# laboshinl/loam_velodyne

Hardware: AMD Instinct MI355X
Metric: sweeps/sec (64-ring, 1M-pt map): feature extraction + odometry + scan-to-map registration (higher is better)
Workload: dtype f32

## Files before the change

### loam_velodyne_amd/csrc/features.hip

```cpp
#include "features.hpp"
#include "pinned_copy.hpp"
#include "scan.hpp"

namespace loamx {

__device__ inline float sqdiff3(const float4& a, const float4& b) {
  const float dx = a.x - b.x, dy = a.y - b.y, dz = a.z - b.z;
  return dx * dx + dy * dy + dz * dz;
}
__device__ inline float sqdiff3w(const float4& a, const float4& b, float wb) {
  const float dx = a.x - b.x * wb, dy = a.y - b.y * wb, dz = a.z - b.z * wb;
  return dx * dx + dy * dy + dz * dz;
}

struct RingLds {
  uint8_t* flags;
  float* c;
  uint32_t* sorted;
  int8_t* label;
};

__device__ inline void wave_lds_sync() { __builtin_amdgcn_fence(__ATOMIC_ACQ_REL, "workgroup"); }

__device__ inline void mark_as_picked(uint32_t scan_i, int cr, uint8_t* flags, const uint8_t* gaps, int lane) {
  bool brk = false;
  if (lane < cr) brk = gaps[scan_i + lane] != 0;
  else if (lane >= 32 && lane < 32 + cr) brk = gaps[scan_i - (lane - 32) - 1] != 0;
  const unsigned long long m = __ballot(brk);
  const uint32_t mf = (uint32_t)(m & 0xffffffffull), mb = (uint32_t)(m >> 32);
  const int nf = mf ? __builtin_ctz(mf) : cr;
  const int nb = mb ? __builtin_ctz(mb) : cr;
  if (lane == 0) flags[scan_i] = 1;
  if (lane < nf) flags[scan_i + lane + 1] = 1;
  if (lane >= 32 && lane - 32 < nb) flags[scan_i - (lane - 32) - 1] = 1;
  wave_lds_sync();
}

__device__ inline void mark_as_picked_split(uint32_t scan_i, int cr, uint8_t* flags, uint8_t* fwd, const uint8_t* gaps, int lane, uint32_t r_lo,
                                            uint32_t r_hi) {
  bool brk = false;
  if (lane < cr) brk = gaps[scan_i + lane] != 0;
  else if (lane >= 32 && lane < 32 + cr) brk = gaps[scan_i - (lane - 32) - 1] != 0;
  const unsigned long long m = __ballot(brk);
  const uint32_t mf = (uint32_t)(m & 0xffffffffull), mb = (uint32_t)(m >> 32);
  const int nf = mf ? __builtin_ctz(mf) : cr;
  const int nb = mb ? __builtin_ctz(mb) : cr;
  if (lane == 0) flags[scan_i] = 1;
  if (lane < nf) {
    const uint32_t t = scan_i + lane + 1;
    if (t < r_hi) flags[t] = 1;
    else fwd[t] = 1;
  }
  if (lane >= 32 && lane - 32 < nb) {
    const uint32_t t = scan_i - (lane - 32) - 1;
    if (t >= r_lo) flags[t] = 1;
  }
  wave_lds_sync();
}

__device__ inline void region_picks(const FeatParams& P, int cr, uint32_t rn, uint32_t rgsp, uint32_t rscan, const float* rc, const uint32_t* rsorted,
                                    int8_t* rlabel, uint8_t* flags, uint8_t* fwd, const uint8_t* gaps, uint32_t* outS, uint32_t* outLS, uint32_t* outF,
                                    uint32_t* cnt3, int lane) {
  const uint32_t r_lo = rscan, r_hi = rscan + rn;
  uint32_t nS = 0, nLS = 0, nF = 0;
  {
    int picked = 0;
    int pos = (int)rn;
    while (pos > 0 && picked < P.max_less_sharp) {
      const int kk = pos - 1 - lane;
      const bool in = kk >= 0;
      const uint32_t e = in ? rsorted[kk] : 0u;
      const float ce = in ? rc[e] : 0.f;
      const bool above = in && (ce > P.curv_thr);
      const bool ok = above && flags[rscan + e] == 0;
      const unsigned long long mok = __ballot(ok), mstop = __ballot(in && !above);
      const int fo = mok ? __builtin_ctzll(mok) : 64, fs = mstop ? __builtin_ctzll(mstop) : 64;
      if (fo < fs) {
        const uint32_t pe = __shfl(e, fo, 64);
        picked++;
        if (lane == 0) {
          if (picked <= P.max_sharp) {
            rlabel[pe] = 2;
            outS[nS] = rgsp + pe;
          } else {
            rlabel[pe] = 1;
          }
          outLS[nLS] = rgsp + pe;
        }
        if (picked <= P.max_sharp) nS++;
        nLS++;
        if (fwd) mark_as_picked_split(rscan + pe, cr, flags, fwd, gaps, lane, r_lo, r_hi);
        else mark_as_picked(rscan + pe, cr, flags, gaps, lane);
        pos = pos - 1 - fo;
      } else if (fs < 64) {
        break;
      } else {
        pos -= 64;
      }
    }
  }
  {
    int picked = 0;
    int pos = 0;
    while (pos < (int)rn && picked < P.max_flat) {
      const int kk = pos + lane;
      const bool in = kk < (int)rn;
      const uint32_t e = in ? rsorted[kk] : 0u;
      const float ce = in ? rc[e] : 0.f;
      const bool below = in && (ce < P.curv_thr);
      const bool ok = below && flags[rscan + e] == 0;
      const unsigned long long mok = __ballot(ok), mstop = __ballot(in && !below);
      const int fo = mok ? __builtin_ctzll(mok) : 64, fs = mstop ? __builtin_ctzll(mstop) : 64;
      if (fo < fs) {
        const uint32_t pe = __shfl(e, fo, 64);
        picked++;
        if (lane == 0) {
          rlabel[pe] = -1;
          outF[nF] = rgsp + pe;
        }
        nF++;
        if (fwd) mark_as_picked_split(rscan + pe, cr, flags, fwd, gaps, lane, r_lo, r_hi);
        else mark_as_picked(rscan + pe, cr, flags, gaps, lane);
        pos = pos + fo + 1;
      } else if (fs < 64) {
        break;
      } else {
        pos += 64;
      }
    }
  }
  if (lane == 0) { cnt3[0] = nS; cnt3[1] = nLS; cnt3[2] = nF; }
  wave_lds_sync();
}

template <int KPL>
__device__ inline void wave_sort_curvature(const float* __restrict__ c, uint32_t n, uint32_t* __restrict__ sorted, int lane) {
  unsigned long long a[KPL];
#pragma unroll
  for (int r = 0; r < KPL; r++) {
    const uint32_t e = (uint32_t)(r * 64 + lane);
    a[r] = e < n ? ((unsigned long long)__float_as_uint(c[e]) << 32) | e : ~0ull;
  }
  constexpr uint32_t N = 64u * KPL;
#pragma nounroll
  for (uint32_t k = 2; k <= N; k <<= 1) {
#pragma nounroll
    for (uint32_t j = k >> 1; j >= (uint32_t)KPL; j >>= 1) {
      const int pl = (int)(j / KPL);
      const bool lower = (lane & pl) == 0;
#pragma unroll
      for (int r = 0; r < KPL; r++) {
        const unsigned long long x = a[r];
        const unsigned long long y = __shfl_xor(x, pl, 64);
        const uint32_t i = (uint32_t)lane * KPL + (uint32_t)r;
// ... 141 lines not shown
        if (!(ep > sp) || ep - sp + 1 < (unsigned long long)cr) simple = 0;
      }
      s_simple = simple && !force_sequential;
    }
    float* c = (float*)(wave_base + wid * wave_bytes);
    uint32_t* sorted = (uint32_t*)(c + nmax);
    int8_t* label = (int8_t*)(sorted + nmax);
    for (int jb = 0; jb < nreg; jb += FEAT_WAVES) {
      const int j = jb + wid;
      uint32_t n = 0, gsp = 0, scan_sp = 0;
      if (j < nreg) {
        const unsigned long long sp = ((s0 + cr) * (unsigned long long)(nreg - j) + (e0 - cr) * (unsigned long long)j) / nreg;
        const unsigned long long ep = ((s0 + cr) * (unsigned long long)(nreg - 1 - j) + (e0 - cr) * (unsigned long long)(j + 1)) / nreg - 1;
        if (ep > sp) {
          n = (uint32_t)(ep - sp + 1);
          gsp = base + (uint32_t)sp;
          scan_sp = (uint32_t)(sp - s0);
        }
      }
      if (lane == 0) { reg_n[wid] = n; reg_gsp[wid] = gsp; reg_scan[wid] = scan_sp; }
      for (uint32_t e = lane; e < n; e += 64) {
        c[e] = curv_all[scan_sp + e];
        label[e] = 0;
      }
      if (lane < 4 && n) c[n + lane] = __builtin_inff();
      __syncthreads();
      FT_TS(1);
      if (sortP == 64) wave_sort_curvature<1>(c, n, sorted, lane);
      else if (sortP == 128) wave_sort_curvature<2>(c, n, sorted, lane);
      else if (sortP == 256) wave_sort_curvature<4>(c, n, sorted, lane);
      else if (sortP == 512) wave_sort_curvature<8>(c, n, sorted, lane);
      else if (wid < (int)nwaves) {
        unsigned long long* keys = (unsigned long long*)(wave_base + nwaves * wave_bytes + (size_t)wid * sortP * 8);
        for (uint32_t e = lane; e < sortP; e += 64)
          keys[e] = e < n ? ((unsigned long long)__float_as_uint(c[e]) << 32) | e : ~0ull;
        wave_lds_sync();
        for (uint32_t k = 2; k <= sortP; k <<= 1) {
          for (uint32_t j = k >> 1; j > 0; j >>= 1) {
            for (uint32_t t = lane; t < sortP / 2; t += 64) {
              const uint32_t i = ((t / j) * 2 * j) + (t % j), l = i + j;
              const unsigned long long a = keys[i], b = keys[l];
              const bool up = (i & k) == 0;
              if ((a > b) == up) { keys[i] = b; keys[l] = a; }
            }
            wave_lds_sync();
          }
        }
        for (uint32_t e = lane; e < n; e += 64) sorted[e] = (uint32_t)keys[e];
      }
      __syncthreads();
      FT_TS(2);
      if (s_simple) {
        const uint32_t rn = reg_n[wid];
        if (rn) {
          if (wid == 0 && jb > 0)
            for (uint32_t e = lane; e < (uint32_t)cr && e < rn; e += 64) flags[reg_scan[0] + e] |= fwd[reg_scan[0] + e];
          wave_lds_sync();
          region_picks(P, cr, rn, reg_gsp[wid], reg_scan[wid], c, sorted, label, flags, fwd, gaps, pickS + (size_t)j * P.max_sharp,
                       pickLS + (size_t)j * P.max_less_sharp, pickF + (size_t)j * P.max_flat, rcnt[j], lane);
        }
        __syncthreads();
        if (wid == 0) {
          for (int w = 1; w < FEAT_WAVES && jb + w < nreg; w++) {
            const uint32_t rn2 = reg_n[w], rscan2 = reg_scan[w], rgsp2 = reg_gsp[w];
            const float* rc = (const float*)(wave_base + w * wave_bytes);
            const uint32_t* rsorted = (const uint32_t*)(rc + nmax);
            int8_t* rlabel = (int8_t*)(rsorted + nmax);
            const bool hit = lane < cr && (uint32_t)lane < rn2 && fwd[rscan2 + lane] != 0 && rlabel[lane] != 0;
            if (__ballot(hit)) {
              for (uint32_t e = lane; e < rn2; e += 64) {
                flags[rscan2 + e] = flags0[rscan2 + e] | (e < (uint32_t)cr ? fwd[rscan2 + e] : (uint8_t)0);
                rlabel[e] = 0;
              }
              for (uint32_t e = lane; e < (uint32_t)cr; e += 64) fwd[rscan2 + rn2 + e] = 0;
              wave_lds_sync();
              region_picks(P, cr, rn2, rgsp2, rscan2, rc, rsorted, rlabel, flags, fwd, gaps, pickS + (size_t)(jb + w) * P.max_sharp,
                           pickLS + (size_t)(jb + w) * P.max_less_sharp, pickF + (size_t)(jb + w) * P.max_flat, rcnt[jb + w], lane);
            }
          }
        }
      } else if (wid == 0) {
        for (int w = 0; w < FEAT_WAVES && jb + w < nreg; w++) {
          const uint32_t rn2 = reg_n[w];
          if (rn2 == 0) continue;
          const float* rc = (const float*)(wave_base + w * wave_bytes);
          const uint32_t* rsorted = (const uint32_t*)(rc + nmax);
          int8_t* rlabel = (int8_t*)(rsorted + nmax);
          region_picks(P, cr, rn2, reg_gsp[w], reg_scan[w], rc, rsorted, rlabel, flags, nullptr, gaps, pickS + (size_t)(jb + w) * P.max_sharp,
                       pickLS + (size_t)(jb + w) * P.max_less_sharp, pickF + (size_t)(jb + w) * P.max_flat, rcnt[jb + w], lane);
        }
      }
      __syncthreads();
      FT_TS(3);
      for (uint32_t e = lane; e < n; e += 64) lf_valid[gsp + e] = label[e] <= 0 ? 1 : 0;
      __syncthreads();
    }
  }
  if (wid == 0 && len > 2u * cr + 1u) {
    uint32_t* lists[3] = {pickS, pickLS, pickF};
    const uint32_t per[3] = {(uint32_t)P.max_sharp, (uint32_t)P.max_less_sharp, (uint32_t)P.max_flat};
    uint32_t tot[3] = {0, 0, 0};
    for (int j = 0; j < nreg; j++) {
#pragma unroll
      for (int q = 0; q < 3; q++) {
        const uint32_t cnt = rcnt[j][q], src = (uint32_t)j * per[q];
        if (src != tot[q]) {
          for (uint32_t k0 = 0; k0 < cnt; k0 += 64) {
            const uint32_t k = k0 + lane;
            const uint32_t v = k < cnt ? lists[q][src + k] : 0u;
            wave_lds_sync();
            if (k < cnt) lists[q][tot[q] + k] = v;
            wave_lds_sync();
          }
        }
        tot[q] += cnt;
      }
    }
    nS = tot[0]; nLS = tot[1]; nF = tot[2];
  }
  if (tid == 0) {
    cntS[r] = nS;
    cntLS[r] = nLS;
    cntF[r] = nF;
    npick[0] = nS; npick[1] = nLS; npick[2] = nF;
  }
  __syncthreads();
  for (uint32_t k = tid; k < npick[0]; k += blockDim.x) slotS[(size_t)r * capS + k] = cloud[pickS[k]];
  for (uint32_t k = tid; k < npick[1]; k += blockDim.x) slotLS[(size_t)r * capLS + k] = cloud[pickLS[k]];
  for (uint32_t k = tid; k < npick[2]; k += blockDim.x) slotF[(size_t)r * capF + k] = cloud[pickF[k]];
  FT_TS(4);
}

struct FeatRingLds {
  uint32_t flag_bytes, nmax, sortP, nwaves;
  size_t bytes;
};
constexpr size_t FEAT_LDS_STATIC = 1024;
constexpr size_t FEAT_LDS_MAX = 160 * 1024 - FEAT_LDS_STATIC;
static_assert(sizeof(uint32_t) * (3 * FEAT_WAVES + 3 + 64 * 3) + sizeof(int) <= FEAT_LDS_STATIC, "k_feat_ring's static LDS");

static FeatRingLds feat_ring_lds(uint32_t max_len, const FeatParams& p) {
  FeatRingLds r;
  const size_t caps = (size_t)(p.max_sharp + p.max_less_sharp + p.max_flat) * p.n_regions;
  r.flag_bytes = (max_len + 15u) & ~15u;
  r.nmax = (max_len / (uint32_t)p.n_regions + 8u + 15u) & ~15u;
  r.sortP = 64;
  while (r.sortP < r.nmax) r.sortP <<= 1;
  r.nwaves = (uint32_t)std::min(p.n_regions, FEAT_WAVES);
  r.bytes = ((8 * (size_t)r.flag_bytes + 4 * caps + 15) & ~(size_t)15) + (size_t)r.nwaves * r.nmax * (4 + 4 + 1) +
            (r.sortP > 512 ? (size_t)r.nwaves * r.sortP * 8 : 0) + 16;
  return r;
}

constexpr int LFV_THREADS = 1024;
constexpr uint32_t LFV_MAX = 4096;

__global__ __launch_bounds__(LFV_THREADS) void k_feat_lf_voxel(const float4* __restrict__ cloud, const uint32_t* __restrict__ ring_off,
                                                               const uint8_t* __restrict__ lf_valid, float inv_leaf, uint32_t P,
                                                               float4* __restrict__ slots, uint32_t* __restrict__ cnt) {
  extern __shared__ __attribute__((aligned(16))) char smem[];
  unsigned long long* keys = (unsigned long long*)smem;
  __shared__ uint32_t sc[17];
  __shared__ int mm[6];
  __shared__ uint32_t s_wcnt[LFV_THREADS / 64][256];
  __shared__ uint32_t s_base[256];
  const uint32_t r = blockIdx.x, tid = threadIdx.x;
  const uint32_t s0 = ring_off[r], len = ring_off[r + 1] - s0;
  if (tid < 3) mm[tid] = 2147483647;
  else if (tid < 6) mm[tid] = -2147483647 - 1;
  for (uint32_t k = tid; k < P; k += LFV_THREADS) keys[k] = ~0ull;
  __syncthreads();
  uint32_t base = 0;
  for (uint32_t b = 0; b < len; b += LFV_THREADS) {
    const uint32_t i = b + tid;
    const uint32_t v = (i < len && lf_valid[s0 + i]) ? 1u : 0u;
    uint32_t total;
    const uint32_t ex = block_excl_scan(v, sc, total);
    if (v) keys[base + ex] = i;
    base += total;
  }
  const uint32_t m = base;
  __syncthreads();
  {
    int lo[3] = {2147483647, 2147483647, 2147483647}, hi[3] = {-2147483647 - 1, -2147483647 - 1, -2147483647 - 1};
    for (uint32_t j = tid; j < m; j += LFV_THREADS) {
      const float4 p = cloud[s0 + (uint32_t)keys[j]];
      const int c[3] = {(int)floorf(p.x * inv_leaf), (int)floorf(p.y * inv_leaf), (int)floorf(p.z * inv_leaf)};
#pragma unroll
      for (int a = 0; a < 3; a++) { lo[a] = min(lo[a], c[a]); hi[a] = max(hi[a], c[a]); }
    }
#pragma unroll
    for (int off = 32; off > 0; off >>= 1) {
#pragma unroll
      for (int a = 0; a < 3; a++) {
        lo[a] = min(lo[a], __shfl_xor(lo[a], off, 64));
        hi[a] = max(hi[a], __shfl_xor(hi[a], off, 64));
      }
    }
    if ((tid & 63u) == 0) {
#pragma unroll
      for (int a = 0; a < 3; a++) { atomicMin(&mm[a], lo[a]); atomicMax(&mm[3 + a], hi[a]); }
    }
  }
  __syncthreads();
  const long long dx = (long long)mm[3] - mm[0] + 1, dy = (long long)mm[4] - mm[1] + 1, dz = (long long)mm[5] - mm[2] + 1;
  const bool pass = m > 0 && (dx > 2147483647LL || dy > 2147483647LL || dx * dy > 2147483647LL || dz > 2147483647LL / (dx * dy) + 1 || dx * dy * dz > 2147483647LL);
  for (uint32_t j = tid; j < m; j += LFV_THREADS) {
    const uint32_t li = (uint32_t)keys[j];
    unsigned long long k;
    if (pass) {
      k = (unsigned long long)j;
    } else {
      const float4 p = cloud[s0 + li];
      const int jx = (int)floorf(p.x * inv_leaf), jy = (int)floorf(p.y * inv_leaf), jz = (int)floorf(p.z * inv_leaf);
      k = (unsigned long long)((long long)(jx - mm[0]) + (long long)(jy - mm[1]) * dx + (long long)(jz - mm[2]) * dx * dy);
    }
    keys[j] = (k << 12) | li;
  }
  __syncthreads();
  unsigned long long* kb[2] = {keys, (unsigned long long*)(smem + (size_t)P * 8)};
  uint32_t npass = 0;
  if (!pass && m > 1) {
    const unsigned long long top = (unsigned long long)(dx * dy * dz - 1);
    const uint32_t bits = top ? 64u - (uint32_t)__builtin_clzll(top) : 0u;
    npass = (bits + 7u) / 8u;
  }
  {
    const uint32_t lane = tid & 63u, wid = tid >> 6;
    const uint32_t per_wave = ((m + LFV_THREADS - 1) / LFV_THREADS) * 64u;
    for (uint32_t ps = 0; ps < npass; ps++) {
      const uint32_t shift = 12u + 8u * ps;
      const unsigned long long* src = kb[ps & 1];
      unsigned long long* dst = kb[(ps & 1) ^ 1];
      for (uint32_t e = tid; e < (LFV_THREADS / 64) * 256; e += LFV_THREADS) (&s_wcnt[0][0])[e] = 0u;
      __syncthreads();
      unsigned long long key[4];
      uint32_t rank[4];
#pragma unroll
      for (int j = 0; j < 4; j++) {
        const uint32_t i = wid * per_wave + (uint32_t)j * 64u + lane;
        const bool in = (uint32_t)j * 64u < per_wave && i < m;
        key[j] = in ? src[i] : ~0ull;
        const uint32_t d = (uint32_t)((key[j] >> shift) & 255ull);
        unsigned long long mt = __ballot(in);
#pragma unroll
        for (int b = 0; b < 8; b++) {
          const unsigned long long bal = __ballot((d >> b) & 1u);
          mt &= ((d >> b) & 1u) ? bal : ~bal;
        }
        const unsigned long long below = mt & ((1ull << lane) - 1ull);
        const int leader = __builtin_ctzll(mt | (1ull << 63));
        uint32_t old = 0u;
        if (in && (int)lane == leader) {
          old = s_wcnt[wid][d];
          s_wcnt[wid][d] = old + (uint32_t)__popcll(mt);
        }
        old = __shfl(old, leader, 64);
        rank[j] = old + (uint32_t)__popcll(below);
        __builtin_amdgcn_wave_barrier();
      }
      __syncthreads();
      uint32_t run = 0;
      if (tid < 256) {
#pragma unroll
        for (int w = 0; w < LFV_THREADS / 64; w++) { const uint32_t c = s_wcnt[w][tid]; s_wcnt[w][tid] = run; run += c; }
      }
      uint32_t tot;
      const uint32_t ex = block_excl_scan(run, sc, tot);
      if (tid < 256) s_base[tid] = ex;
      __syncthreads();
#pragma unroll
      for (int j = 0; j < 4; j++) {
        const uint32_t i = wid * per_wave + (uint32_t)j * 64u + lane;
        if ((uint32_t)j * 64u < per_wave && i < m) {
          const uint32_t d = (uint32_t)((key[j] >> shift) & 255ull);
          dst[s_base[d] + s_wcnt[wid][d] + rank[j]] = key[j];
        }
      }
      __syncthreads();
    }
    if (npass & 1u) {
      for (uint32_t j = tid; j < m; j += LFV_THREADS) keys[j] = kb[1][j];
      __syncthreads();
    }
  }
  float4* sp = (float4*)(smem + (size_t)P * 8);
  for (uint32_t j = tid; j < m; j += LFV_THREADS) sp[j] = cloud[s0 + (uint32_t)(keys[j] & 4095ull)];
  __syncthreads();
  uint32_t obase = 0;
  for (uint32_t b = 0; b < m; b += LFV_THREADS) {
    const uint32_t j = b + tid;
    const bool head = j < m && (j == 0 || (keys[j] >> 12) != (keys[j - 1] >> 12));
    uint32_t total;
    const uint32_t ex = block_excl_scan(head ? 1u : 0u, sc, total);
    if (head) {
      const unsigned long long vk = keys[j] >> 12;
      float sx = 0.f, sy = 0.f, sz = 0.f, si = 0.f;
      uint32_t e = j;
      do {
        const float4 p = sp[e];
        sx += p.x; sy += p.y; sz += p.z; si += p.w;
        e++;
      } while (e < m && (keys[e] >> 12) == vk);
      const float c = (float)(e - j);
      slots[s0 + obase + ex] = make_float4(sx / c, sy / c, sz / c, si / c);
    }
    obase += total;
  }
  if (tid == 0) cnt[r] = obase;
}

__device__ inline uint32_t rings_before(const uint32_t* __restrict__ c, uint32_t r, int lane) {
  uint32_t part = 0u;
  for (uint32_t i = (uint32_t)lane; i < r; i += 64u) part += c[i];
#pragma unroll
  for (int d = 32; d > 0; d >>= 1) part += (uint32_t)__shfl_xor((int)part, d, 64);
  return part;
}
__global__ __launch_bounds__(64) void k_feat_compact(const float4* __restrict__ s0, const float4* __restrict__ s1, const float4* __restrict__ s2,
                                                     const uint32_t* __restrict__ c0, const uint32_t* __restrict__ c1, const uint32_t* __restrict__ c2,
                                                     uint32_t cap0, uint32_t cap1, uint32_t cap2, float4* __restrict__ o0, float4* __restrict__ o1,
                                                     float4* __restrict__ o2, uint32_t* __restrict__ offs, const uint32_t* __restrict__ sweep_ring_base,
                                                     uint32_t nsw, uint32_t* __restrict__ host_offs) {
  const uint32_t r = blockIdx.x, kind = blockIdx.y, nring = gridDim.x;
  const int lane = (int)threadIdx.x;
  const float4* s = kind == 0 ? s0 : (kind == 1 ? s1 : s2);
  const uint32_t* c = kind == 0 ? c0 : (kind == 1 ? c1 : c2);
  const uint32_t cap = kind == 0 ? cap0 : (kind == 1 ? cap1 : cap2);
  float4* o = kind == 0 ? o0 : (kind == 1 ? o1 : o2);
  const uint32_t dst = rings_before(c, r, lane), n = c[r];
  for (uint32_t k = (uint32_t)lane; k < n; k += 64u) o[dst + k] = s[(size_t)r * cap + k];
  if (lane == 0) {
    uint32_t* off = offs + (size_t)kind * (nsw + 1);
    uint32_t* hoff = host_offs ? host_offs + (size_t)kind * (nsw + 1) : nullptr;
    uint32_t lo = 0, hi = nsw + 1;
    while (lo < hi) { const uint32_t mid = (lo + hi) >> 1; if (sweep_ring_base[mid] < r) lo = mid + 1; else hi = mid; }
    for (uint32_t sw = lo; sw <= nsw && sweep_ring_base[sw] == r; sw++) { off[sw] = dst; if (hoff) hoff[sw] = dst; }
    if (r + 1 == nring)
      for (uint32_t sw = nsw; sweep_ring_base[sw] >= nring; sw--) { off[sw] = dst + n; if (hoff) hoff[sw] = dst + n; if (sw == 0) break; }
  }
}
__global__ __launch_bounds__(256) void k_feat_lf_compact(const float4* __restrict__ slots, const uint32_t* __restrict__ ring_off,
                                                         const uint32_t* __restrict__ cnt, uint32_t* __restrict__ lf_off, float4* __restrict__ out,
                                                         uint32_t* __restrict__ host_lf_off) {
  __shared__ uint32_t s_dst;
  const uint32_t r = blockIdx.x;
  if (threadIdx.x < 64) {
    const uint32_t d = rings_before(cnt, r, (int)threadIdx.x);
    if (threadIdx.x == 0) {
      s_dst = d;
      lf_off[r] = d;
      if (r + 1 == gridDim.x) lf_off[gridDim.x] = d + cnt[r];
      if (host_lf_off) {
        host_lf_off[r] = d;
        if (r + 1 == gridDim.x) host_lf_off[gridDim.x] = d + cnt[r];
      }
    }
  }
  __syncthreads();
  const uint32_t n = cnt[r], src = ring_off[r], dst = s_dst;
  for (uint32_t k = threadIdx.x; k < n; k += blockDim.x) out[dst + k] = slots[src + k];
}

FeatureExtractor::FeatureExtractor(int device, hipStream_t shared_stream) : device_(device) {
  select_device(device);
  if (shared_stream) {
    st_ = shared_stream;
  } else {
    LX_HIP(hipStreamCreateWithFlags(&st_, hipStreamNonBlocking));
    own_stream_ = true;
  }
  vox_.init(st_);
  h_bad_.reserve(16);
  h_bad_.p[0] = 0u;
  h_bad_.p[1] = 0u;
}

void FeatureExtractor::check_finite_input() {
  if (*(volatile uint32_t*)h_bad_.p) {
    *h_bad_.p = 0u;
    throw Error(LOAMX_E_INVALID, "a sweep holds non-finite coordinates (binned rings must be finite: BasicLaserOdometry.cpp:230 / MultiScanRegistration.cpp:187-196 drop such points before this stage)");
  }
}

FeatureExtractor::~FeatureExtractor() {
  if (ev_front_) (void)hipEventDestroy(ev_front_);
  if (ev_lf_) (void)hipEventDestroy(ev_lf_);
  if (own_stream_ && st_) (void)hipStreamDestroy(st_);
}

void FeatureExtractor::check_params_() const {
  LX_REQUIRE(params.curv_region >= 1 && params.curv_region <= 16, "curvature_region must be in [1,16]");
  LX_REQUIRE(params.n_regions >= 1 && params.n_regions <= 64, "n_feature_regions must be in [1,64]");
  LX_REQUIRE(params.max_sharp >= 0 && params.max_flat >= 0 && params.max_less_sharp >= params.max_sharp, "invalid pick limits");
  LX_REQUIRE(params.less_flat_leaf > 0.f, "less_flat_filter_size must be positive");
}

void FeatureExtractor::upload_async(uint32_t nsw, const loamx_cloud* clouds, const uint32_t* const* ring_size, const uint32_t* n_rings,
                                    hipStream_t copy_stream, hipEvent_t done, const std::function<bool(void*, const void*, size_t)>& big_copy) {
  LX_REQUIRE(nsw >= 1 && clouds && ring_size && n_rings && copy_stream && done, "invalid sweep batch");
  check_params_();
  LX_HIP(hipSetDevice(device_));
  bool packed = true;
  for (uint32_t s = 0; s < nsw; s++) {
    check_cloud(&clouds[s], false);
    uint32_t sum = 0;
    for (uint32_t r = 0; r < n_rings[s]; r++) sum += ring_size[s][r];
    LX_REQUIRE(sum == clouds[s].count, "ring sizes do not add up to the cloud size");
    packed = packed && clouds[s].stride == 16 && clouds[s].intensity_offset == 12;
  }
  layout_(nsw, ring_size, n_rings);
  allocate_(copy_stream);
  if (packed) {
    for (uint32_t s = 0; s < nsw;) {
      uint32_t e = s + 1;
      size_t cnt = clouds[s].count;
      while (e < nsw && (const char*)clouds[e].data == (const char*)clouds[s].data + sizeof(float4) * cnt) cnt += clouds[e++].count;
      if (cnt && !(big_copy && big_copy(cloud_.p + h_pt_base_[s], clouds[s].data, sizeof(float4) * cnt)))
        LX_HIP(hipMemcpyAsync(cloud_.p + h_pt_base_[s], clouds[s].data, sizeof(float4) * cnt, hipMemcpyHostToDevice, copy_stream));
      s = e;
    }
  } else {
    h_cloud_.reserve(n_ + 1);
    for (uint32_t s = 0; s < nsw; s++) pack_cloud(&clouds[s], h_cloud_.p + h_pt_base_[s]);
    if (n_) LX_HIP(hipMemcpyAsync(cloud_.p, h_cloud_.p, sizeof(float4) * n_, hipMemcpyHostToDevice, copy_stream));
  }
  LX_HIP(hipEventRecord(done, copy_stream));
}
void FeatureExtractor::upload_device(uint32_t nsw, const float4* d_src, const uint32_t* src_off, const uint32_t* const* ring_size,
                                     const uint32_t* n_rings, hipStream_t copy_stream, hipEvent_t done) {
  LX_REQUIRE(nsw >= 1 && d_src && src_off && ring_size && n_rings && copy_stream && done, "invalid sweep batch");
  check_params_();
  LX_HIP(hipSetDevice(device_));
  layout_(nsw, ring_size, n_rings);
  allocate_(copy_stream);
  for (uint32_t s = 0; s < nsw; s++) {
    const uint32_t cnt = h_pt_base_[s + 1] - h_pt_base_[s];
    if (cnt) LX_HIP(hipMemcpyAsync(cloud_.p + h_pt_base_[s], d_src + src_off[s], sizeof(float4) * cnt, hipMemcpyDeviceToDevice, copy_stream));
  }
  LX_HIP(hipEventRecord(done, copy_stream));
}
void FeatureExtractor::layout_(uint32_t nsw, const uint32_t* const* ring_size, const uint32_t* n_rings) {
  uint32_t longest = 0;
  for (uint32_t s = 0; s < nsw; s++)
    for (uint32_t r = 0; r < n_rings[s]; r++) longest = std::max(longest, ring_size[s][r]);
  LX_REQUIRE(feat_ring_lds(longest, params).bytes <= FEAT_LDS_MAX, "scan ring too long for the LDS staging of k_feat_ring (include/loamx.h)");
  nsw_ = nsw;
  h_ring_off_.assign(1, 0);
  h_ring_base_.assign(nsw + 1, 0);
  h_pt_base_.assign(nsw + 1, 0);
  h_ring_sweep_base_.clear();
  max_ring_len_ = 0;
  uint32_t pt = 0;
  for (uint32_t s = 0; s < nsw; s++) {
    uint32_t sum = 0;
    for (uint32_t r = 0; r < n_rings[s]; r++) {
      sum += ring_size[s][r];
      h_ring_off_.push_back(pt + sum);
      h_ring_sweep_base_.push_back(pt);
      max_ring_len_ = std::max(max_ring_len_, ring_size[s][r]);
    }
    pt += sum;
// ... 123 lines not shown
    h_imu_d_.reserve(2 * (size_t)H);
    h_imu_f_.reserve(9 * (size_t)H);
    imu_.fill_table(h_imu_d_.p, h_imu_f_.p, I);
    imu_dt_.reserve(2 * (size_t)H);
    imu_state_.reserve(9 * (size_t)H);
    imu_last_.reserve(1);
    h_imu_last_.reserve(1);
    LX_HIP(hipMemcpyAsync(imu_dt_.p, h_imu_d_.p, sizeof(double) * 2 * H, hipMemcpyHostToDevice, st_));
    LX_HIP(hipMemcpyAsync(imu_state_.p, h_imu_f_.p, sizeof(float) * 9 * H, hipMemcpyHostToDevice, st_));
    LX_HIP(hipMemsetAsync(imu_last_.p, 0, sizeof(ImuLast), st_));
    I.dt = imu_dt_.p;
    I.dstamp = imu_dt_.p + H;
    I.state = imu_state_.p;
  }
  return H;
}

void FeatureExtractor::finish_raw_(uint32_t n_scan_rings, uint32_t H) {
  LX_HIP(hipMemcpyAsync(h_raw_ring_cnt_.p, raw_ring_cnt_.p, sizeof(uint32_t) * n_scan_rings, hipMemcpyDeviceToHost, st_));
  if (H) LX_HIP(hipMemcpyAsync(h_imu_last_.p, imu_last_.p, sizeof(ImuLast), hipMemcpyDeviceToHost, st_));
  LX_HIP(hipStreamSynchronize(st_));
  if (H && h_imu_last_.p->valid) imu_.apply_last(*h_imu_last_.p);
  begin_sweep();
  const uint32_t* rs[1] = {h_raw_ring_cnt_.p};
  layout_(1, rs, &n_scan_rings);
  allocate_();
  LX_HIP(hipStreamSynchronize(st_));
}

void ImuTracker::update(double stamp, float roll, float pitch, float yaw, const float acc_in[3]) {
  State st;
  st.stamp = stamp; st.roll = HAngle(roll); st.pitch = HAngle(pitch); st.yaw = HAngle(yaw);
  st.acceleration = {acc_in[0], acc_in[1], acc_in[2]};
  if (!hist_.empty()) {
    HVec3 acc = st.acceleration;
    h_rot_zxy(acc, st.roll, st.pitch, st.yaw);
    const State& prev = hist_.back();
    const float dt = (float)(stamp - prev.stamp);
    st.position = {prev.position.x + prev.velocity.x * dt + 0.5f * acc.x * dt * dt, prev.position.y + prev.velocity.y * dt + 0.5f * acc.y * dt * dt,
                   prev.position.z + prev.velocity.z * dt + 0.5f * acc.z * dt * dt};
    st.velocity = {prev.velocity.x + acc.x * dt, prev.velocity.y + acc.y * dt, prev.velocity.z + acc.z * dt};
  }
  if (hist_.size() >= (size_t)std::max(history_size, 1)) hist_.pop_front();
  hist_.push_back(st);
}

void ImuTracker::interpolate_for_(float rel, State& out) {
  double td = (scan_time_ - hist_[idx_].stamp) + rel;
  while (idx_ < hist_.size() - 1 && td > 0) {
    idx_++;
    td = (scan_time_ - hist_[idx_].stamp) + rel;
  }
  if (idx_ == 0 || td > 0) {
    out = hist_[idx_];
  } else {
    const State &a = hist_[idx_], &b = hist_[idx_ - 1];
    const float ratio = (float)(-td / (a.stamp - b.stamp)), inv = 1 - ratio;
    out.roll = HAngle(a.roll.r * inv + b.roll.r * ratio);
    out.pitch = HAngle(a.pitch.r * inv + b.pitch.r * ratio);
    if (a.yaw.r - b.yaw.r > M_PI) out.yaw = HAngle((float)(a.yaw.r * inv + (b.yaw.r + 2 * M_PI) * ratio));
    else if (a.yaw.r - b.yaw.r < -M_PI) out.yaw = HAngle((float)(a.yaw.r * inv + (b.yaw.r - 2 * M_PI) * ratio));
    else out.yaw = HAngle(a.yaw.r * inv + b.yaw.r * ratio);
    out.velocity = {a.velocity.x * inv + b.velocity.x * ratio, a.velocity.y * inv + b.velocity.y * ratio, a.velocity.z * inv + b.velocity.z * ratio};
    out.position = {a.position.x * inv + b.position.x * ratio, a.position.y * inv + b.position.y * ratio, a.position.z * inv + b.position.z * ratio};
  }
}

void ImuTracker::begin_sweep() {
  scan_time_ = next_scan_time_;
  idx_ = 0;
  if (!hist_.empty()) interpolate_for_(0.f, start_);
  sweep_start_ = scan_time_;
  imu_trans_[0] = start_.pitch.r; imu_trans_[1] = start_.yaw.r; imu_trans_[2] = start_.roll.r;
  imu_trans_[3] = cur_.pitch.r; imu_trans_[4] = cur_.yaw.r; imu_trans_[5] = cur_.roll.r;
  HVec3 sh = shift_;
  h_rot_yxz(sh, -start_.yaw, -start_.pitch, -start_.roll);
  imu_trans_[6] = sh.x; imu_trans_[7] = sh.y; imu_trans_[8] = sh.z;
  HVec3 v{cur_.velocity.x - start_.velocity.x, cur_.velocity.y - start_.velocity.y, cur_.velocity.z - start_.velocity.z};
  h_rot_yxz(v, -start_.yaw, -start_.pitch, -start_.roll);
  imu_trans_[9] = v.x; imu_trans_[10] = v.y; imu_trans_[11] = v.z;
}

void ImuTracker::fill_table(double* h_d, float* h_f, ImuTable& I) const {
  const uint32_t H = (uint32_t)hist_.size();
  for (uint32_t j = 0; j < H; j++) {
    const State& s = hist_[j];
    h_d[j] = scan_time_ - s.stamp;
    h_d[H + j] = j ? s.stamp - hist_[j - 1].stamp : 1.0;
    float* o = h_f + 9 * (size_t)j;
    o[0] = s.roll.r; o[1] = s.pitch.r; o[2] = s.yaw.r;
    o[3] = s.position.x; o[4] = s.position.y; o[5] = s.position.z;
    o[6] = s.velocity.x; o[7] = s.velocity.y; o[8] = s.velocity.z;
  }
  I.H = H;
  I.idx0 = H ? (uint32_t)std::min(idx_, (size_t)H - 1) : 0u;
  const HAngle* sa[3] = {&start_.roll, &start_.pitch, &start_.yaw};
  for (int k = 0; k < 3; k++) { I.start_c[k] = sa[k]->c; I.start_s[k] = sa[k]->s; }
  I.start_pos[0] = start_.position.x; I.start_pos[1] = start_.position.y; I.start_pos[2] = start_.position.z;
  I.start_vel[0] = start_.velocity.x; I.start_vel[1] = start_.velocity.y; I.start_vel[2] = start_.velocity.z;
  I.rel_sweep_base = scan_time_ - sweep_start_;
}

void ImuTracker::apply_last(const ImuLast& L) {
  cur_.roll = HAngle(L.roll); cur_.pitch = HAngle(L.pitch); cur_.yaw = HAngle(L.yaw);
  cur_.position = {L.pos[0], L.pos[1], L.pos[2]};
  cur_.velocity = {L.vel[0], L.vel[1], L.vel[2]};
  shift_ = {L.shift[0], L.shift[1], L.shift[2]};
  idx_ = L.idx;
}

int FeatureExtractor::download_cloud(uint32_t sweep, loamx_cloud* full, uint32_t* ring_size_out) {
  LX_REQUIRE(sweep < nsw_, "sweep index out of range");
  const uint32_t r0 = h_ring_base_[sweep], r1 = h_ring_base_[sweep + 1];
  if (ring_size_out)
    for (uint32_t r = r0; r < r1; r++) ring_size_out[r - r0] = h_ring_off_[r + 1] - h_ring_off_[r];
  if (!full) return LOAMX_OK;
  check_cloud(full, false);
  const uint32_t a = h_pt_base_[sweep], b = h_pt_base_[sweep + 1];
  h_pack_.reserve((size_t)(b - a) + 2);
  if (b > a) LX_HIP(hipMemcpyAsync(h_pack_.p, cloud_.p + a, sizeof(float4) * (b - a), hipMemcpyDeviceToHost, st_));
  LX_HIP(hipStreamSynchronize(st_));
  return unpack_cloud(h_pack_.p, b - a, full);
}

void FeatureExtractor::run_async(bool mirror_offsets) {
  TraceRange trace_range("loamx:features:extract");
  LX_REQUIRE(nsw_ > 0, "run() before upload()");
  LX_HIP(hipSetDevice(device_));
  split_ = mirror_offsets && max_ring_len_ <= LFV_MAX;
  uint32_t* hmir = nullptr;
  if (split_) {
    h_mirror_off_.reserve(n_offsets());
    hmir = h_mirror_off_.p;
    if (!ev_front_) { LX_HIP(hipEventCreateWithFlags(&ev_front_, hipEventDisableTiming)); LX_HIP(hipEventCreateWithFlags(&ev_lf_, hipEventDisableTiming)); }
  }
  const int cr = params.curv_region;
  (void)cr;
  const uint32_t caps[3] = {(uint32_t)(params.max_sharp * params.n_regions), (uint32_t)(params.max_less_sharp * params.n_regions),
                            (uint32_t)(params.max_flat * params.n_regions)};
  const FeatRingLds L = feat_ring_lds(max_ring_len_, params);
  const size_t lds = L.bytes;
  LX_REQUIRE(lds <= FEAT_LDS_MAX, "internal: scan ring too long for the LDS staging of k_feat_ring");
  static const bool force_seq = diag_env("LOAMX_FEAT_SEQUENTIAL") && atoi(diag_env("LOAMX_FEAT_SEQUENTIAL")) != 0;
  if (lds > 64 * 1024)
    LX_HIP(hipFuncSetAttribute((const void*)k_feat_ring, hipFuncAttributeMaxDynamicSharedMemorySize, (int)lds));
  hipLaunchKernelGGL(k_feat_ring, dim3(nring_), dim3(64 * FEAT_WAVES), lds, st_, cloud_.p, ring_off_.p, ring_sweep_base_.p, params, L.flag_bytes, L.nmax,
                     L.sortP, L.nwaves, slots_[0].p, slots_[1].p, slots_[2].p, slot_cnt_[0].p, slot_cnt_[1].p, slot_cnt_[2].p, lf_valid_.p, force_seq ? 1 : 0,
                     h_bad_.p);
  hipLaunchKernelGGL(k_feat_compact, dim3(nring_, 3), dim3(64), 0, st_, slots_[0].p, slots_[1].p, slots_[2].p, slot_cnt_[0].p, slot_cnt_[1].p,
                     slot_cnt_[2].p, caps[0], caps[1], caps[2], out_[0].p, out_[1].p, out_[2].p, offs_.p, sweep_ring_base_.p, nsw_, hmir);
  if (split_) LX_HIP(hipEventRecord(ev_front_, st_));
  const float inv = 1.0f / params.less_flat_leaf;
  if (max_ring_len_ <= LFV_MAX) {
    uint32_t P = 2;
    while (P < max_ring_len_) P <<= 1;
    if ((size_t)P * 24 > 64 * 1024)
      LX_HIP(hipFuncSetAttribute((const void*)k_feat_lf_voxel, hipFuncAttributeMaxDynamicSharedMemorySize, (int)((size_t)P * 24)));
    hipLaunchKernelGGL(k_feat_lf_voxel, dim3(nring_), dim3(LFV_THREADS), (size_t)P * 24, st_, cloud_.p, ring_off_.p, lf_valid_.p, inv, P,
                       lf_slots_.p, lf_cnt_.p);
    hipLaunchKernelGGL(k_feat_lf_compact, dim3(nring_), dim3(256), 0, st_, lf_slots_.p, ring_off_.p, lf_cnt_.p, lf_off_(), lf_out_.p,
                       hmir ? hmir + (size_t)3 * off_stride_ : nullptr);
    if (split_) LX_HIP(hipEventRecord(ev_lf_, st_));
  } else {
    vox_.compute_ijk(cloud_.p, lf_valid_.p, n_, ring_off_.p, nring_, inv, inv);
    vox_.sort_reduce(cloud_.p, lf_valid_.p, n_, ring_off_.p, nring_, lf_out_.p, lf_off_());
  }
#ifdef LOAMX_PROF_FEAT
  {
    unsigned long long ts[8];
    LX_HIP(hipStreamSynchronize(st_));
    LX_HIP(hipMemcpyFromSymbol(ts, HIP_SYMBOL(g_feat_ts), sizeof(ts)));
    fprintf(stderr, "[feat_ring ts, 10ns ticks] load %lld  rank-sort %lld  picks %lld  tail %lld\n", (long long)(ts[1] - ts[0]), (long long)(ts[2] - ts[1]),
            (long long)(ts[3] - ts[2]), (long long)(ts[4] - ts[3]));
  }
#endif
  LX_HIP(hipGetLastError());
}

void FeatureExtractor::sync() {
  LX_HIP(hipStreamSynchronize(st_));
  vox_.check();
  check_finite_input();
}

__global__ __launch_bounds__(256) void k_feat_pack_host(const float4* __restrict__ o0, const float4* __restrict__ o1, const float4* __restrict__ o2,
                                                        const float4* __restrict__ lf, const uint32_t* __restrict__ off0,
                                                        const uint32_t* __restrict__ off1, const uint32_t* __restrict__ off2,
                                                        const uint32_t* __restrict__ lf_off, uint32_t sweep, uint32_t ring_a, uint32_t ring_b,
                                                        uint32_t capacity, float4* __restrict__ dst) {
  const uint32_t a0 = off0[sweep], n0 = off0[sweep + 1] - a0, a1 = off1[sweep], n1 = off1[sweep + 1] - a1;
  const uint32_t a2 = off2[sweep], n2 = off2[sweep + 1] - a2, a3 = lf_off[ring_a], n3 = lf_off[ring_b] - a3;
  const uint32_t total = n0 + n1 + n2 + n3;
  if (blockIdx.x == 0 && threadIdx.x == 0) {
    uint4 h = make_uint4(n0, n1, n2, n3);
    if (total > capacity) h = make_uint4(0xffffffffu, 0xffffffffu, 0xffffffffu, 0xffffffffu);
    *reinterpret_cast<uint4*>(dst) = h;
  }
  if (total > capacity) return;
  for (uint32_t i = blockIdx.x * blockDim.x + threadIdx.x; i < total; i += gridDim.x * blockDim.x) {
    float4 v;
    if (i < n0) v = o0[a0 + i];
    else if (i < n0 + n1) v = o1[a1 + (i - n0)];
    else if (i < n0 + n1 + n2) v = o2[a2 + (i - n0 - n1)];
    else v = lf[a3 + (i - n0 - n1 - n2)];
    dst[1 + i] = v;
  }
}

void FeatureExtractor::device_results(uint32_t sweep, const float4* ptr[4], uint32_t count[4]) {
  LX_REQUIRE(sweep < nsw_, "sweep index out of range");
  h_link_off_.reserve(n_offsets());
  LX_HIP(hipMemcpyAsync(h_link_off_.p, offs_.p, sizeof(uint32_t) * n_offsets(), hipMemcpyDeviceToHost, st_));
  LX_HIP(hipStreamSynchronize(st_));
  vox_.check();
  check_finite_input();
  const uint32_t* o = h_link_off_.p;
  for (int k = 0; k < 3; k++) {
    const uint32_t a = o[(size_t)k * off_stride_ + sweep], b = o[(size_t)k * off_stride_ + sweep + 1];
    ptr[k] = out_[k].p + a;
    count[k] = b - a;
  }
  const uint32_t* lf = o + (size_t)3 * off_stride_;
  const uint32_t a = lf[h_ring_base_[sweep]], b = lf[h_ring_base_[sweep + 1]];
  ptr[3] = lf_out_.p + a;
  count[3] = b - a;
}

void FeatureExtractor::device_results_front(uint32_t sweep, const float4* ptr[3], uint32_t count[3]) {
  LX_REQUIRE(sweep < nsw_, "sweep index out of range");
  LX_REQUIRE(split_, "internal: device_results_front() without run_async(true)");
  spin_event(ev_front_);
  check_finite_input();
  const uint32_t* o = h_mirror_off_.p;
  for (int k = 0; k < 3; k++) {
    const uint32_t a = o[(size_t)k * off_stride_ + sweep], b = o[(size_t)k * off_stride_ + sweep + 1];
    ptr[k] = out_[k].p + a;
    count[k] = b - a;
  }
}
void FeatureExtractor::device_results_lf(uint32_t sweep, const float4*& ptr, uint32_t& count) {
  LX_REQUIRE(sweep < nsw_, "sweep index out of range");
  LX_REQUIRE(split_, "internal: device_results_lf() without run_async(true)");
  spin_event(ev_lf_);
  const uint32_t* lf = h_mirror_off_.p + (size_t)3 * off_stride_;
  const uint32_t a = lf[h_ring_base_[sweep]], b = lf[h_ring_base_[sweep + 1]];
  ptr = lf_out_.p + a;
  count = b - a;
}

int FeatureExtractor::download(uint32_t sweep, loamx_cloud* sharp, loamx_cloud* less_sharp, loamx_cloud* flat, loamx_cloud* less_flat) {
  LX_REQUIRE(sweep < nsw_, "sweep index out of range");
  loamx_cloud* outs[4] = {sharp, less_sharp, flat, less_flat};
  for (auto* o : outs) if (o) check_cloud(o, false);
  const uint32_t n_pts = h_pt_base_[sweep + 1] - h_pt_base_[sweep];
  const uint32_t capacity = 4 * n_pts;
  h_pack_.reserve((size_t)capacity + 2);
  hipLaunchKernelGGL(k_feat_pack_host, dim3(std::min<uint32_t>((capacity + 1023) / 1024 + 1, 128u)), dim3(256), 0, st_, out_[0].p, out_[1].p, out_[2].p,
                     lf_out_.p, d_feat_off(0), d_feat_off(1), d_feat_off(2), lf_off_(), sweep, h_ring_base_[sweep], h_ring_base_[sweep + 1], capacity,
                     h_pack_.p);
  LX_HIP(hipStreamSynchronize(st_));
  vox_.check();
  check_finite_input();
  const uint32_t* hdr = reinterpret_cast<const uint32_t*>(h_pack_.p);
  LX_REQUIRE(hdr[0] != 0xffffffffu, "internal: the feature clouds of a sweep exceed four times its points");
  int rc = LOAMX_OK;
  const float4* src = h_pack_.p + 1;
  for (int k = 0; k < 4; k++) {
    if (outs[k]) {
      const int r = unpack_cloud(src, hdr[k], outs[k]);
      if (r != LOAMX_OK) rc = r;
    }
    src += hdr[k];
  }
  return rc;
}

}
```

Measured before the change: 16240.

## Rework less-flat voxel kernel around register-resident keys and shared ring radix pass

Rewrites k_feat_lf_voxel so each thread holds eight points in registers. Points are loaded once into LDS staging, voxel coordinates are computed once, and keys stay in registers through each radix pass. A reusable ring_radix_pass uses 16-bit per-wave counters and a single-wave scan, and the block size is sized to the ring length (P/8, at most 512) rather than fixed at 1024. Voxel means are computed per thread over contiguous runs, with a tail walk for runs that cross thread boundaries. This cuts redundant global reloads, the compaction scan and barriers, at the cost of more complex boundary logic and an extra sort pass when all keys fit in one.

Measured after the change: 16610, median of 3. +2.3%, better.

```diff
diff --git a/loam_velodyne_amd/csrc/features.hip b/loam_velodyne_amd/csrc/features.hip
--- a/loam_velodyne_amd/csrc/features.hip
+++ b/loam_velodyne_amd/csrc/features.hip
@@ -1,5 +1,6 @@
 #include "features.hpp"
 #include "pinned_copy.hpp"
+#include "ring_radix.hpp"
 #include "scan.hpp"
 
 namespace loamx {
@@ -447,42 +448,60 @@
   return r;
 }
 
-constexpr int LFV_THREADS = 1024;
-constexpr uint32_t LFV_MAX = 4096;
-
-__global__ __launch_bounds__(LFV_THREADS) void k_feat_lf_voxel(const float4* __restrict__ cloud, const uint32_t* __restrict__ ring_off,
-                                                               const uint8_t* __restrict__ lf_valid, float inv_leaf, uint32_t P,
-                                                               float4* __restrict__ slots, uint32_t* __restrict__ cnt) {
+constexpr int LFV_MAX_THREADS = 512;
+constexpr uint32_t LFV_MAX = 4096, LFV_MIN_P = 512;
+static_assert(LFV_MAX / 8 == LFV_MAX_THREADS && LFV_MAX_THREADS / 64 <= RR_MAX_WAVES, "k_feat_lf_voxel: eight elements per thread");
+
+#ifdef LOAMX_PROF_LFV
+__device__ unsigned long long g_lfv_ts[8];
+#define LFV_TS(k) do { if (blockIdx.x == gridDim.x / 2 && threadIdx.x == 0) g_lfv_ts[k] = wall_clock64(); } while (0)
+#else
+#define LFV_TS(k) do { } while (0)
+#endif
+
+__global__ __launch_bounds__(LFV_MAX_THREADS) void k_feat_lf_voxel(const float4* __restrict__ cloud, const uint32_t* __restrict__ ring_off,
+                                                                   const uint8_t* __restrict__ lf_valid, float inv_leaf, uint32_t P,
+                                                                   float4* __restrict__ slots, uint32_t* __restrict__ cnt) {
   extern __shared__ __attribute__((aligned(16))) char smem[];
-  unsigned long long* keys = (unsigned long long*)smem;
+  float4* stage = (float4*)smem;
+  unsigned long long* s_w = (unsigned long long*)(smem + (size_t)P * 16);
+  __shared__ RingRadixLds s_rx;
   __shared__ uint32_t sc[17];
   __shared__ int mm[6];
-  __shared__ uint32_t s_wcnt[LFV_THREADS / 64][256];
-  __shared__ uint32_t s_base[256];
-  const uint32_t r = blockIdx.x, tid = threadIdx.x;
+  const uint32_t r = blockIdx.x, tid = threadIdx.x, lane = tid & 63u, wid = tid >> 6;
   const uint32_t s0 = ring_off[r], len = ring_off[r + 1] - s0;
   if (tid < 3) mm[tid] = 2147483647;
   else if (tid < 6) mm[tid] = -2147483647 - 1;
-  for (uint32_t k = tid; k < P; k += LFV_THREADS) keys[k] = ~0ull;
-  __syncthreads();
-  uint32_t base = 0;
-  for (uint32_t b = 0; b < len; b += LFV_THREADS) {
-    const uint32_t i = b + tid;
-    const uint32_t v = (i < len && lf_valid[s0 + i]) ? 1u : 0u;
-    uint32_t total;
-    const uint32_t ex = block_excl_scan(v, sc, total);
-    if (v) keys[base + ex] = i;
-    base += total;
-  }
-  const uint32_t m = base;
-  __syncthreads();
+  LFV_TS(0);
+  int vx[8], vy[8], vz[8];
+  uint32_t cand = 0u;
+  {
+    float4 pt[8];
+    uint8_t ok[8];
+#pragma unroll
+    for (int j = 0; j < 8; j++) {
+      const uint32_t i = wid * 512u + (uint32_t)j * 64u + lane;
+      pt[j] = i < len ? cloud[s0 + i] : make_float4(0.f, 0.f, 0.f, 0.f);
+      ok[j] = i < len ? lf_valid[s0 + i] : (uint8_t)0;
+    }
+#pragma unroll
+    for (int j = 0; j < 8; j++) {
+      const uint32_t i = wid * 512u + (uint32_t)j * 64u + lane;
+      if (i < len) stage[i] = pt[j];
+      cand |= ok[j] ? (1u << j) : 0u;
+      vx[j] = (int)floorf(pt[j].x * inv_leaf); vy[j] = (int)floorf(pt[j].y * inv_leaf); vz[j] = (int)floorf(pt[j].z * inv_leaf);
+    }
+  }
+  LFV_TS(1);
   {
     int lo[3] = {2147483647, 2147483647, 2147483647}, hi[3] = {-2147483647 - 1, -2147483647 - 1, -2147483647 - 1};
-    for (uint32_t j = tid; j < m; j += LFV_THREADS) {
-      const float4 p = cloud[s0 + (uint32_t)keys[j]];
-      const int c[3] = {(int)floorf(p.x * inv_leaf), (int)floorf(p.y * inv_leaf), (int)floorf(p.z * inv_leaf)};
-#pragma unroll
-      for (int a = 0; a < 3; a++) { lo[a] = min(lo[a], c[a]); hi[a] = max(hi[a], c[a]); }
+#pragma unroll
+    for (int j = 0; j < 8; j++) {
+      if ((cand >> j) & 1u) {
+        lo[0] = min(lo[0], vx[j]); hi[0] = max(hi[0], vx[j]);
+        lo[1] = min(lo[1], vy[j]); hi[1] = max(hi[1], vy[j]);
+        lo[2] = min(lo[2], vz[j]); hi[2] = max(hi[2], vz[j]);
+      }
     }
 #pragma unroll
     for (int off = 32; off > 0; off >>= 1) {
@@ -492,117 +511,112 @@
         hi[a] = max(hi[a], __shfl_xor(hi[a], off, 64));
       }
     }
-    if ((tid & 63u) == 0) {
+    __syncthreads();
+    if (lane == 0 && lo[0] <= hi[0]) {
 #pragma unroll
       for (int a = 0; a < 3; a++) { atomicMin(&mm[a], lo[a]); atomicMax(&mm[3 + a], hi[a]); }
     }
   }
   __syncthreads();
+  LFV_TS(2);
+  if (mm[3] < mm[0]) {
+    if (tid == 0) cnt[r] = 0u;
+    return;
+  }
   const long long dx = (long long)mm[3] - mm[0] + 1, dy = (long long)mm[4] - mm[1] + 1, dz = (long long)mm[5] - mm[2] + 1;
-  const bool pass = m > 0 && (dx > 2147483647LL || dy > 2147483647LL || dx * dy > 2147483647LL || dz > 2147483647LL / (dx * dy) + 1 || dx * dy * dz > 2147483647LL);
-  for (uint32_t j = tid; j < m; j += LFV_THREADS) {
-    const uint32_t li = (uint32_t)keys[j];
-    unsigned long long k;
-    if (pass) {
-      k = (unsigned long long)j;
-    } else {
-      const float4 p = cloud[s0 + li];
-      const int jx = (int)floorf(p.x * inv_leaf), jy = (int)floorf(p.y * inv_leaf), jz = (int)floorf(p.z * inv_leaf);
-      k = (unsigned long long)((long long)(jx - mm[0]) + (long long)(jy - mm[1]) * dx + (long long)(jz - mm[2]) * dx * dy);
-    }
-    keys[j] = (k << 12) | li;
-  }
-  __syncthreads();
-  unsigned long long* kb[2] = {keys, (unsigned long long*)(smem + (size_t)P * 8)};
-  uint32_t npass = 0;
-  if (!pass && m > 1) {
+  const bool pass = dx > 2147483647LL || dy > 2147483647LL || dx * dy > 2147483647LL || dz > 2147483647LL / (dx * dy) + 1 || dx * dy * dz > 2147483647LL;
+  unsigned long long w[8];
+#pragma unroll
+  for (int j = 0; j < 8; j++) {
+    const uint32_t i = wid * 512u + (uint32_t)j * 64u + lane;
+    unsigned long long k = 0ull;
+    if (!pass && ((cand >> j) & 1u)) k = (unsigned long long)((long long)(vx[j] - mm[0]) + (long long)(vy[j] - mm[1]) * dx + (long long)(vz[j] - mm[2]) * dx * dy);
+    w[j] = ((cand >> j) & 1u) ? ((k << 12) | (unsigned long long)i) : RR_NONE;
+  }
+  uint32_t npass = 1u;
+  if (!pass) {
     const unsigned long long top = (unsigned long long)(dx * dy * dz - 1);
     const uint32_t bits = top ? 64u - (uint32_t)__builtin_clzll(top) : 0u;
-    npass = (bits + 7u) / 8u;
-  }
+    npass = max((bits + 7u) / 8u, 1u);
+  }
+  uint32_t m = 0u;
+  for (uint32_t ps = 0; ps < npass; ps++) {
+    m = ring_radix_pass(w, 12u + 8u * ps, s_w, s_rx);
+    if (ps + 1u < npass) {
+#pragma unroll
+      for (int j = 0; j < 8; j++) {
+        const uint32_t i = wid * 512u + (uint32_t)j * 64u + lane;
+        w[j] = i < m ? s_w[i] : RR_NONE;
+      }
+    }
+    LFV_TS(3 + (ps < 3u ? ps : 3u));
+  }
+  const uint32_t l0 = tid * 8u;
+  unsigned long long vox[8];
+  float4 pt[8];
+  bool head[8];
+  uint32_t nh = 0u;
   {
-    const uint32_t lane = tid & 63u, wid = tid >> 6;
-    const uint32_t per_wave = ((m + LFV_THREADS - 1) / LFV_THREADS) * 64u;
-    for (uint32_t ps = 0; ps < npass; ps++) {
-      const uint32_t shift = 12u + 8u * ps;
-      const unsigned long long* src = kb[ps & 1];
-      unsigned long long* dst = kb[(ps & 1) ^ 1];
-      for (uint32_t e = tid; e < (LFV_THREADS / 64) * 256; e += LFV_THREADS) (&s_wcnt[0][0])[e] = 0u;
-      __syncthreads();
-      unsigned long long key[4];
-      uint32_t rank[4];
-#pragma unroll
-      for (int j = 0; j < 4; j++) {
-        const uint32_t i = wid * per_wave + (uint32_t)j * 64u + lane;
-        const bool in = (uint32_t)j * 64u < per_wave && i < m;
-        key[j] = in ? src[i] : ~0ull;
-        const uint32_t d = (uint32_t)((key[j] >> shift) & 255ull);
-        unsigned long long mt = __ballot(in);
-#pragma unroll
-        for (int b = 0; b < 8; b++) {
-          const unsigned long long bal = __ballot((d >> b) & 1u);
-          mt &= ((d >> b) & 1u) ? bal : ~bal;
-        }
-        const unsigned long long below = mt & ((1ull << lane) - 1ull);
-        const int leader = __builtin_ctzll(mt | (1ull << 63));
-        uint32_t old = 0u;
-        if (in && (int)lane == leader) {
-          old = s_wcnt[wid][d];
-          s_wcnt[wid][d] = old + (uint32_t)__popcll(mt);
-        }
-        old = __shfl(old, leader, 64);
-        rank[j] = old + (uint32_t)__popcll(below);
-        __builtin_amdgcn_wave_barrier();
-      }
-      __syncthreads();
-      uint32_t run = 0;
-      if (tid < 256) {
-#pragma unroll
-        for (int w = 0; w < LFV_THREADS / 64; w++) { const uint32_t c = s_wcnt[w][tid]; s_wcnt[w][tid] = run; run += c; }
-      }
-      uint32_t tot;
-      const uint32_t ex = block_excl_scan(run, sc, tot);
-      if (tid < 256) s_base[tid] = ex;
-      __syncthreads();
-#pragma unroll
-      for (int j = 0; j < 4; j++) {
-        const uint32_t i = wid * per_wave + (uint32_t)j * 64u + lane;
-        if ((uint32_t)j * 64u < per_wave && i < m) {
-          const uint32_t d = (uint32_t)((key[j] >> shift) & 255ull);
-          dst[s_base[d] + s_wcnt[wid][d] + rank[j]] = key[j];
-        }
-      }
-      __syncthreads();
-    }
-    if (npass & 1u) {
-      for (uint32_t j = tid; j < m; j += LFV_THREADS) keys[j] = kb[1][j];
-      __syncthreads();
-    }
-  }
-  float4* sp = (float4*)(smem + (size_t)P * 8);
-  for (uint32_t j = tid; j < m; j += LFV_THREADS) sp[j] = cloud[s0 + (uint32_t)(keys[j] & 4095ull)];
-  __syncthreads();
-  uint32_t obase = 0;
-  for (uint32_t b = 0; b < m; b += LFV_THREADS) {
-    const uint32_t j = b + tid;
-    const bool head = j < m && (j == 0 || (keys[j] >> 12) != (keys[j - 1] >> 12));
-    uint32_t total;
-    const uint32_t ex = block_excl_scan(head ? 1u : 0u, sc, total);
-    if (head) {
-      const unsigned long long vk = keys[j] >> 12;
-      float sx = 0.f, sy = 0.f, sz = 0.f, si = 0.f;
-      uint32_t e = j;
-      do {
-        const float4 p = sp[e];
-        sx += p.x; sy += p.y; sz += p.z; si += p.w;
-        e++;
-      } while (e < m && (keys[e] >> 12) == vk);
-      const float c = (float)(e - j);
-      slots[s0 + obase + ex] = make_float4(sx / c, sy / c, sz / c, si / c);
-    }
-    obase += total;
-  }
-  if (tid == 0) cnt[r] = obase;
+    unsigned long long prev = (l0 == 0u || l0 >= m) ? RR_NONE : (s_w[l0 - 1u] >> 12);
+#pragma unroll
+    for (int j = 0; j < 8; j++) {
+      const uint32_t l = l0 + (uint32_t)j;
+      const unsigned long long x = l < m ? s_w[l] : RR_NONE;
+      vox[j] = x >> 12;
+      pt[j] = stage[l < m ? (uint32_t)(x & 4095ull) : 0u];
+      head[j] = l < m && (pass || l == 0u || vox[j] != prev);
+      nh += head[j] ? 1u : 0u;
+      prev = vox[j];
+    }
+  }
+  const unsigned long long nextv = (l0 + 8u < m ? s_w[l0 + 8u] : RR_NONE) >> 12;
+  uint32_t tot;
+  uint32_t pos = s0 + block_excl_scan(nh, sc, tot);
+  float lx = 0.f, ly = 0.f, lz = 0.f, li = 0.f;
+  uint32_t lcnt = 0u, lpos = 0u;
+  unsigned long long lvox = RR_NONE;
+#pragma unroll
+  for (int j = 0; j < 8; j++) {
+    if (head[j]) {
+      float sx = 0.f + pt[j].x, sy = 0.f + pt[j].y, sz = 0.f + pt[j].z, si = 0.f + pt[j].w;
+      uint32_t cntp = 1u;
+      bool open = !pass;
+#pragma unroll
+      for (int q = j + 1; q < 8; q++) {
+        open = open && vox[q] == vox[j];
+        if (open) { sx += pt[q].x; sy += pt[q].y; sz += pt[q].z; si += pt[q].w; cntp++; }
+      }
+      if (open && nextv == vox[j]) {
+        lx = sx; ly = sy; lz = sz; li = si; lcnt = cntp; lpos = pos; lvox = vox[j];
+      } else {
+        const float c = (float)cntp;
+        slots[pos] = make_float4(sx / c, sy / c, sz / c, si / c);
+      }
+      pos++;
+    }
+  }
+  if (lcnt) {
+    uint32_t l = l0 + 8u;
+    bool open = true;
+    while (open) {
+      unsigned long long xs[8];
+      float4 ts[8];
+#pragma unroll
+      for (int q = 0; q < 8; q++) xs[q] = l + (uint32_t)q < m ? s_w[l + (uint32_t)q] : RR_NONE;
+#pragma unroll
+      for (int q = 0; q < 8; q++) ts[q] = stage[xs[q] != RR_NONE ? (uint32_t)(xs[q] & 4095ull) : 0u];
+#pragma unroll
+      for (int q = 0; q < 8; q++) {
+        open = open && (xs[q] >> 12) == lvox;
+        if (open) { lx += ts[q].x; ly += ts[q].y; lz += ts[q].z; li += ts[q].w; lcnt++; }
+      }
+      l += 8u;
+    }
+    const float c = (float)lcnt;
+    slots[lpos] = make_float4(lx / c, ly / c, lz / c, li / c);
+  }
+  if (tid == 0) cnt[r] = tot;
+  LFV_TS(7);
 }
 
 __device__ inline uint32_t rings_before(const uint32_t* __restrict__ c, uint32_t r, int lane) {
@@ -1032,11 +1046,11 @@
   if (split_) LX_HIP(hipEventRecord(ev_front_, st_));
   const float inv = 1.0f / params.less_flat_leaf;
   if (max_ring_len_ <= LFV_MAX) {
-    uint32_t P = 2;
+    uint32_t P = LFV_MIN_P;
     while (P < max_ring_len_) P <<= 1;
     if ((size_t)P * 24 > 64 * 1024)
       LX_HIP(hipFuncSetAttribute((const void*)k_feat_lf_voxel, hipFuncAttributeMaxDynamicSharedMemorySize, (int)((size_t)P * 24)));
-    hipLaunchKernelGGL(k_feat_lf_voxel, dim3(nring_), dim3(LFV_THREADS), (size_t)P * 24, st_, cloud_.p, ring_off_.p, lf_valid_.p, inv, P,
+    hipLaunchKernelGGL(k_feat_lf_voxel, dim3(nring_), dim3(P / 8), (size_t)P * 24, st_, cloud_.p, ring_off_.p, lf_valid_.p, inv, P,
                        lf_slots_.p, lf_cnt_.p);
     hipLaunchKernelGGL(k_feat_lf_compact, dim3(nring_), dim3(256), 0, st_, lf_slots_.p, ring_off_.p, lf_cnt_.p, lf_off_(), lf_out_.p,
                        hmir ? hmir + (size_t)3 * off_stride_ : nullptr);
@@ -1052,6 +1066,16 @@
     LX_HIP(hipMemcpyFromSymbol(ts, HIP_SYMBOL(g_feat_ts), sizeof(ts)));
     fprintf(stderr, "[feat_ring ts, 10ns ticks] load %lld  rank-sort %lld  picks %lld  tail %lld\n", (long long)(ts[1] - ts[0]), (long long)(ts[2] - ts[1]),
             (long long)(ts[3] - ts[2]), (long long)(ts[4] - ts[3]));
+  }
+#endif
+#ifdef LOAMX_PROF_LFV
+  if (max_ring_len_ <= LFV_MAX) {
+    unsigned long long ts[8];
+    LX_HIP(hipStreamSynchronize(st_));
+    LX_HIP(hipMemcpyFromSymbol(ts, HIP_SYMBOL(g_lfv_ts), sizeof(ts)));
+    fprintf(stderr, "[feat_lf_voxel ts, 10ns ticks since start] load %lld  bounds %lld  pass0 %lld  pass1 %lld  pass2 %lld  pass3 %lld  means %lld  (a pass that did not run shows an old stamp)\n",
+            (long long)(ts[1] - ts[0]), (long long)(ts[2] - ts[0]), (long long)(ts[3] - ts[0]), (long long)(ts[4] - ts[0]), (long long)(ts[5] - ts[0]),
+            (long long)(ts[6] - ts[0]), (long long)(ts[7] - ts[0]));
   }
 #endif
   LX_HIP(hipGetLastError());
diff --git a/loam_velodyne_amd/csrc/ring_radix.hpp b/loam_velodyne_amd/csrc/ring_radix.hpp
--- /dev/null
+++ b/loam_velodyne_amd/csrc/ring_radix.hpp
@@ -0,0 +1,78 @@
+#pragma once
+#include <hip/hip_runtime.h>
+#include <cstdint>
+
+namespace loamx {
+
+constexpr int RR_MAX_WAVES = 8;
+constexpr unsigned long long RR_NONE = ~0ull;
+
+struct alignas(16) RingRadixLds {
+  uint16_t wcnt[RR_MAX_WAVES][256];
+  uint16_t base[256];
+  uint32_t total;
+};
+
+__device__ inline uint32_t ring_radix_pass(const unsigned long long (&w)[8], uint32_t shift, unsigned long long* __restrict__ dst, RingRadixLds& S) {
+  const int tid = (int)threadIdx.x, lane = tid & 63, wid = tid >> 6, nw = (int)(blockDim.x >> 6);
+  for (int e = tid; e < nw * 128; e += (int)blockDim.x) ((uint32_t*)&S.wcnt[0][0])[e] = 0u;
+  __syncthreads();
+  uint32_t rank[8];
+#pragma unroll
+  for (int j = 0; j < 8; j++) {
+    rank[j] = 0u;
+    const bool in = w[j] != RR_NONE;
+    unsigned long long m = __ballot(in);
+    if (m == 0ull) continue;
+    const uint32_t d = (uint32_t)((w[j] >> shift) & 255ull);
+#pragma unroll
+    for (int bit = 0; bit < 8; bit++) {
+      const unsigned long long bal = __ballot((d >> bit) & 1u);
+      m &= ((d >> bit) & 1u) ? bal : ~bal;
+    }
+    const unsigned long long below = m & ((1ull << lane) - 1ull);
+    const int leader = __builtin_ctzll(m | (1ull << 63));
+    uint32_t old = 0u;
+    if (in && lane == leader) {
+      old = S.wcnt[wid][d];
+      S.wcnt[wid][d] = (uint16_t)(old + (uint32_t)__popcll(m));
+    }
+    old = (uint32_t)__shfl((int)old, leader, 64);
+    rank[j] = old + (uint32_t)__popcll(below);
+    __builtin_amdgcn_wave_barrier();
+  }
+  __syncthreads();
+  if (wid == 0) {
+    uint32_t run[4] = {0u, 0u, 0u, 0u};
+    for (int k = 0; k < nw; k++) {
+      ushort4* p = (ushort4*)&S.wcnt[k][4 * lane];
+      const ushort4 c = *p;
+      *p = make_ushort4((unsigned short)run[0], (unsigned short)run[1], (unsigned short)run[2], (unsigned short)run[3]);
+      run[0] += c.x; run[1] += c.y; run[2] += c.z; run[3] += c.w;
+    }
+    const uint32_t mine = run[0] + run[1] + run[2] + run[3];
+    uint32_t inc = mine;
+#pragma unroll
+    for (int dd = 1; dd < 64; dd <<= 1) {
+      const uint32_t o = (uint32_t)__shfl_up((int)inc, dd, 64);
+      if (lane >= dd) inc += o;
+    }
+    const uint32_t ex = inc - mine;
+    *(ushort4*)&S.base[4 * lane] = make_ushort4((unsigned short)ex, (unsigned short)(ex + run[0]), (unsigned short)(ex + run[0] + run[1]),
+                                                (unsigned short)(ex + run[0] + run[1] + run[2]));
+    if (lane == 63) S.total = inc;
+  }
+  __syncthreads();
+#pragma unroll
+  for (int j = 0; j < 8; j++) {
+    if (w[j] != RR_NONE) {
+      const uint32_t d = (uint32_t)((w[j] >> shift) & 255ull);
+      dst[(uint32_t)S.base[d] + (uint32_t)S.wcnt[wid][d] + rank[j]] = w[j];
+    }
+  }
+  const uint32_t total = S.total;
+  __syncthreads();
+  return total;
+}
+
+}
```
